# HorizonRobotics/HoloAgent

Measured on AMD Instinct MI355X. Metric: HMSG frames/sec (one scene per GPU: map A1-A2, fusion A3-A5, merge A6, pooling A7, floors A8, rooms by the device watershed N1, room clouds, room embeddings and View nodes A9, objects with the view <-> object test A10 and graph assembly A11, nothing handed in -- plus 1000 coarse-to-fine retrieval qu, higher is better.
Workload: dtype f64 geometry / f32 features

## Files before the change

### holoagent_amd/csrc/hmsg_merge.hip

```cpp
#include "hmsg_boundary.h"
#include "hmsg_cloudops.h"

#include <algorithm>
#include <cmath>
#include <numeric>
#include <chrono>
#include <unordered_map>
#include <condition_variable>
#include <deque>
#include <mutex>
#include <thread>

namespace {

struct Cloud {
    long long off = 0;
    int n = 0;
    double mn[3] = {0, 0, 0}, mx[3] = {0, 0, 0};
    bool fixed = false;
    bool fresh = true;
    bool raw = false;
    bool anchor = false;
    unsigned long long uid = 0;
    unsigned id = 0;
// ... 419 lines not shown
        if (lane == 0 && local) atomicAdd(&counts[npairs + lo], local);
    }
}

static const int CAT_CHUNK = 512;
__global__ void k_concat(const double* __restrict__ pool, const CatSeg* __restrict__ segs, int nsegs, double* __restrict__ dst,
                         const unsigned char* __restrict__ poolcore, unsigned char* __restrict__ dstcore, int chunk) {
    const CatSeg sg = segs[find_entry(segs, nsegs, blockIdx.x)];
    const long long p0 = (long long)(blockIdx.x - (unsigned)sg.blk0) * chunk, p1 = min((long long)sg.n, p0 + chunk);
    for (long long i = p0 * 3 + threadIdx.x; i < p1 * 3; i += blockDim.x) dst[sg.dst * 3 + i] = pool[sg.src * 3 + i];
    if (dstcore)
        for (long long i = p0 + threadIdx.x; i < p1; i += blockDim.x)
            dstcore[sg.dst + i] = sg.anchor ? poolcore[sg.src + i] : (unsigned char)0;
}

__host__ __device__ inline double box_iou(const double* amn, const double* amx, const double* bmn, const double* bmx) {
    if (amx[0] <= bmn[0] || bmx[0] <= amn[0] || amx[1] <= bmn[1] || bmx[1] <= amn[1] || amx[2] <= bmn[2] || bmx[2] <= amn[2])
        return 0.0;
    double ov = 1, va = 1, vb = 1;
    for (int k = 0; k < 3; ++k) {
        const double omin = amn[k] < bmn[k] ? bmn[k] : amn[k], omax = bmx[k] < amx[k] ? bmx[k] : amx[k];
        const double d = omax - omin;
        ov *= d < 0.0 ? 0.0 : d;
        va *= amx[k] - amn[k];
        vb *= bmx[k] - bmn[k];
    }
    return ov / (va + vb - ov);
}

static const int GP_TILE = 256;
struct GpTile {
    int row0, gend;
};
template <bool FILL>
__global__ void __launch_bounds__(GP_TILE) k_gp_pairs(const double* __restrict__ box, const GpTile* __restrict__ tiles, double iou_thresh, int n,
                                                      unsigned* __restrict__ cnt, const unsigned* __restrict__ start, int* __restrict__ out,
                                                      long long cap) {
    __shared__ double sb[GP_TILE * 6];
    const GpTile t = tiles[blockIdx.x];
    const int i = t.row0 + (int)threadIdx.x;
    const bool row = i < t.gend;
    double a[6] = {0, 0, 0, 0, 0, 0};
    if (row)
// ... 73 lines not shown
            h_out.ensure(2 + 2 * (size_t)cap_pairs);
        }
    }
    static bool fits(const int* group_off, int n_groups) {
        unsigned long long worst = 0;
        for (int g = 0; g < n_groups; ++g) {
            const unsigned long long m = (unsigned long long)(group_off[g + 1] - group_off[g]);
            worst += m * (m ? m - 1 : 0) / 2;
        }
        return worst < (1ull << 32);
    }
};

double bbox_iou(const Cloud& a, const Cloud& b) {
    return box_iou(a.mn, a.mx, b.mn, b.mx);
}

#define HMSG_BOX_MASK_BODY                                                                                          \
    for (int j = 0; j < n; ++j)                                                                                     \
        cm[j] = (unsigned char)!((q[1] <= lo0[j]) | (hi0[j] <= q[0]) | (q[3] <= lo1[j]) | (hi1[j] <= q[2]) |        \
                                 (q[5] <= lo2[j]) | (hi2[j] <= q[4]));
#if !defined(__HIP_DEVICE_COMPILE__) && defined(__x86_64__)
__attribute__((target("avx2"))) void box_mask_avx2(int n, const double* lo0, const double* hi0, const double* lo1,
                                                   const double* hi1, const double* lo2, const double* hi2, const double* q,
                                                   unsigned char* cm) {
    HMSG_BOX_MASK_BODY
}
#endif
void box_mask(int n, const double* lo0, const double* hi0, const double* lo1, const double* hi1, const double* lo2,
              const double* hi2, const double* q, unsigned char* cm) {
#if !defined(__HIP_DEVICE_COMPILE__) && defined(__x86_64__)
    static const bool have_avx2 = __builtin_cpu_supports("avx2");
    if (have_avx2) {
        box_mask_avx2(n, lo0, hi0, lo1, hi1, lo2, hi2, q, cm);
        return;
    }
#endif
    HMSG_BOX_MASK_BODY
}

struct IntSpan {
    const int* b;
    const int* e;
    size_t size() const { return (size_t)(e - b); }
    int operator[](size_t k) const { return b[k]; }
    const int* begin() const { return b; }
    const int* end() const { return e; }
};
struct CompList {
    std::vector<int> off, mem;
    size_t size() const { return off.empty() ? 0 : off.size() - 1; }
    IntSpan operator[](size_t c) const { return IntSpan{mem.data() + off[c], mem.data() + off[c + 1]}; }
};
// ... 304 lines not shown
        hipLaunchKernelGGL(k_ov_count, dim3(nblk), dim3(256), 0, s, (const double*)pool.p, (const OvGrid*)ds.p, (int)spec.size(),
                           d_cursor.p, ix_cells_used, OVI_CHUNK);
        HMSG_CHECK_LAUNCH();
        hmsg_scan_u32(d_cursor.p, ix_cells.p + ix_cells_used, (size_t)ncell_new, s, ops.scan_tmp, nullptr);
        hipLaunchKernelGGL(k_ov_fill, dim3(nblk), dim3(256), 0, s, (const double*)pool.p, (const OvGrid*)ds.p, (int)spec.size(),
                           (const unsigned*)ix_cells.p, d_cursor.p, ix_cells_used, ix_pts.p, OVI_CHUNK);
        HMSG_CHECK_LAUNCH();
    }

    void overlap_ratios(const std::vector<Cloud>& L, const std::vector<std::pair<int, int>>& pairs, std::vector<double>& ratio,
                        double decide_th, std::vector<unsigned char>* second_ran = nullptr) {
        ratio.assign(pairs.size(), 0.0);
        if (second_ran) second_ran->assign(pairs.size(), 0);
        if (pairs.empty()) return;
        const size_t P = pairs.size();
        std::vector<int> slot(L.size(), -1);
        std::vector<OvGrid> g;
        std::vector<OvTask> tasks(P * 2);
        unsigned nblk1 = 0, nblk2 = 0;
        for (size_t k = 0; k < P; ++k) {
            int a = pairs[k].first, b = pairs[k].second;
            for (int v : {a, b})
                if (slot[v] < 0) {
                    slot[v] = (int)g.size();
                    push_grids(L[v], g);
                }
            if (L[a].n > L[b].n) std::swap(a, b);
            tasks[k] = OvTask{slot[a], slot[b], 0, (int)nblk1};
            tasks[P + k] = OvTask{slot[b], slot[a], L[a].n, (int)nblk2};
            nblk1 += cdiv((size_t)L[a].n, OV_CHUNK);
            nblk2 += cdiv((size_t)L[b].n, OV_CHUNK);
        }
        for (size_t k = 0; k < P; ++k) tasks[P + k].blk0 += (int)nblk1;
// ... 5 lines not shown
        const size_t off_t = (g.size() * sizeof(OvGrid) + 15) & ~(size_t)15, off_c = off_t + tasks.size() * sizeof(OvTask),
                     off_b = off_c + tasks.size() * 4, pack = off_b + nblk_tab * 4;
        h_ovpack.ensure(pack);
        d_ovpack.ensure(pack);
        memcpy(h_ovpack.p, g.data(), g.size() * sizeof(OvGrid));
        memcpy(h_ovpack.p + off_t, tasks.data(), tasks.size() * sizeof(OvTask));
        memset(h_ovpack.p + off_c, 0, tasks.size() * 4);
        {
            int* bt = (int*)(h_ovpack.p + off_b);
            for (size_t k = 0; k < (plan ? P : 2 * P); ++k) {
                const size_t e = k + 1 < 2 * P ? (size_t)tasks[k + 1].blk0 : nblk;
                for (size_t b = (size_t)tasks[k].blk0; b < e; ++b) bt[b] = (int)k;
            }
        }
        upload_pinned(d_ovpack.p, h_ovpack.p, pack, s);
        const OvGrid* const dg = (const OvGrid*)d_ovpack.p;
        const OvTask* const dt = (const OvTask*)(d_ovpack.p + off_t);
        unsigned* const dc = (unsigned*)(d_ovpack.p + off_c);
        const int* const db = (const int*)(d_ovpack.p + off_b);
        const float r = (float)reach;
        const float r2 = (float)(radius * radius);
        const size_t prof_idx = ops.prof->ev.size();
        static const int ov_sorted_src = getenv("HMSG_OV_POOL_ORDER") == nullptr ? 1 : 0;
        unsigned long long* d_ovstat = nullptr;
        if (want_stats) {
            if (!ovstat.p) {
                ovstat.alloc(16);
                HIP_TRY(hipMemsetAsync(ovstat.p, 0, 128, s));
            }
            d_ovstat = ovstat.p;
// ... 73 lines not shown
                        gp_box[(size_t)i * 6 + a] = L[i].n ? L[i].mn[a] : 1e300;
                        gp_box[(size_t)i * 6 + 3 + a] = L[i].n ? L[i].mx[a] : -1e300;
                    }
                long long np = 0;
                const int* pr = gp.run(s, ops.scan_tmp, ops.prof, gp_box.data(), n, group_off->data(), G, iou_thresh, &np);
                for (long long k = 0; k < np; ++k) candidate(pr[2 * k], pr[2 * k + 1]);
            } else {
                for (int g = 0; g < G; ++g)
                    for (int i = (*group_off)[g]; i < (*group_off)[g + 1]; ++i)
                        for (int j = i + 1; j < (*group_off)[g + 1]; ++j) consider(i, j);
            }
        } else if (use_cache) {
            for (int i = 0; i < n; ++i)
                for (int j = i + 1; j < n; ++j) consider(i, j);
        } else {
            std::vector<double>* lo = fp_lo;
            std::vector<double>* hi = fp_hi;
            for (int a = 0; a < 3; ++a) {
                lo[a].resize((size_t)n);
                hi[a].resize((size_t)n);
            }
            fp_fr.resize((size_t)n);
            fp_cand.assign((size_t)n + 8, 0);
            std::vector<unsigned char>& fr = fp_fr;
            double u[6] = {1e300, -1e300, 1e300, -1e300, 1e300, -1e300};
            for (int j = 0; j < n; ++j) {
                fr[(size_t)j] = L[j].fresh ? 1 : 0;
                for (int a = 0; a < 3; ++a) {
                    lo[a][(size_t)j] = L[j].n ? L[j].mn[a] : 1e300;
                    hi[a][(size_t)j] = L[j].n ? L[j].mx[a] : -1e300;
                }
                if (fr[(size_t)j] && L[j].n)
                    for (int a = 0; a < 3; ++a) {
                        u[2 * a] = std::min(u[2 * a], L[j].mn[a]);
                        u[2 * a + 1] = std::max(u[2 * a + 1], L[j].mx[a]);
                    }
            }
            if (!(u[0] <= u[1])) return;
            box_mask(n, lo[0].data(), hi[0].data(), lo[1].data(), hi[1].data(), lo[2].data(), hi[2].data(), u, fp_cand.data());
            fp_sub.clear();
            for (int j = 0; j < n; ++j)
                if (fp_cand[(size_t)j]) fp_sub.push_back(j);
            const int m = (int)fp_sub.size();
            for (int a = 0; a < 3; ++a) {
                fp_slo[a].resize((size_t)m);
                fp_shi[a].resize((size_t)m);
                for (int q = 0; q < m; ++q) {
                    fp_slo[a][(size_t)q] = lo[a][(size_t)fp_sub[(size_t)q]];
                    fp_shi[a][(size_t)q] = hi[a][(size_t)fp_sub[(size_t)q]];
                }
            }
            fp_cand.assign((size_t)m + 8, 0);
            for (int i = 0; i < n; ++i) {
                if (!fr[(size_t)i] || L[i].n == 0) continue;
                unsigned char* cm = fp_cand.data();
                const double q[6] = {lo[0][(size_t)i], hi[0][(size_t)i], lo[1][(size_t)i], hi[1][(size_t)i], lo[2][(size_t)i], hi[2][(size_t)i]};
                box_mask(m, fp_slo[0].data(), fp_shi[0].data(), fp_slo[1].data(), fp_shi[1].data(), fp_slo[2].data(), fp_shi[2].data(), q, cm);
                for (int j0 = 0; j0 < m; j0 += 8) {
                    unsigned long long w;
                    std::memcpy(&w, cm + j0, 8);
                    if (!w) continue;
                    for (int jq = j0; jq < std::min(j0 + 8, m); ++jq) {
                        const int j = fp_sub[(size_t)jq];
                        if (!cm[jq] || j == i || (fr[(size_t)j] && j < i)) continue;
                        consider(std::min(i, j), std::max(i, j));
                    }
                }
            }
        }
    }
    GroupPairs gp;
    std::vector<double> gp_box;
    bool gp_wanted = getenv("HMSG_DEBUG_TREE_HOST_PAIRS") == nullptr;
    double gp_device_batches = 0, gp_host_batches = 0;
    std::vector<double> fp_lo[3], fp_hi[3], fp_slo[3], fp_shi[3];
    std::vector<unsigned char> fp_fr, fp_cand;
    std::vector<int> fp_sub;

    void make_components(const std::vector<Cloud>& L, const std::vector<std::pair<int, int>>& pairs, const std::vector<double>& ratio,
                         const std::vector<std::pair<int, int>>& known_pairs, const std::vector<double>& known, double th,
                         CompList& comps) {
        const int n = (int)L.size();
        std::vector<int> parent(n);
        std::iota(parent.begin(), parent.end(), 0);
        auto find = [&](int x) {
            while (parent[x] != x) x = parent[x] = parent[parent[x]];
            return x;
        };
        auto unite = [&](int a, int b) {
            a = find(a);
            b = find(b);
            if (a != b) parent[std::max(a, b)] = std::min(a, b);
        };
        for (size_t k = 0; k < pairs.size(); ++k) {
            if (use_cache) ratio_cache[L[pairs[k].first].uid * 0x100000000ull + L[pairs[k].second].uid] = ratio[k];
            if (ratio[k] > th) unite(pairs[k].first, pairs[k].second);
        }
        for (size_t k = 0; k < known_pairs.size(); ++k)
            if (known[k] > th) unite(known_pairs[k].first, known_pairs[k].second);
        {
            std::vector<int> comp_of(n, -1), cid(n);
            int nc = 0;
            for (int i = 0; i < n; ++i) {
                int r = find(i);
                if (comp_of[r] < 0) comp_of[r] = nc++;
                cid[i] = comp_of[r];
            }
            comps.off.assign((size_t)nc + 1, 0);
            for (int i = 0; i < n; ++i) ++comps.off[cid[i] + 1];
            for (int c = 0; c < nc; ++c) comps.off[c + 1] += comps.off[c];
            comps.mem.resize(n);
            std::vector<int> cur(comps.off.begin(), comps.off.end() - 1);
            for (int i = 0; i < n; ++i) comps.mem[cur[cid[i]]++] = i;
        }
    }

    std::vector<Cloud> merge_3d_masks(std::vector<Cloud> L, double th, const std::vector<int>* group_off = nullptr,
                                      std::vector<int>* out_group_off = nullptr) {
        const int n = (int)L.size();
        if (out_group_off) out_group_off->assign(group_off->size(), 0);
        if (n == 0) return L;
        auto tnow = [] { return std::chrono::steady_clock::now(); };
        auto t0 = tnow();
        auto lap = [&](int k) {
            auto t1 = tnow();
            tphase[k] += std::chrono::duration<double, std::milli>(t1 - t0).count();
            t0 = t1;
        };
        if (want_stats)
            for (auto& c : L) c.has_index_before = c.has_index;
        build_indices(L);
        lap(0);
        std::vector<std::pair<int, int>> pairs;
        std::vector<double> known;
        std::vector<std::pair<int, int>> known_pairs;
        find_pairs(L, pairs, known, known_pairs, group_off);
        std::vector<double> ratio;
        lap(1);
        std::vector<unsigned char> second_ran;
        overlap_ratios(L, pairs, ratio, use_cache ? -1.0 : th, want_stats ? &second_ran : nullptr);
        lap(2);
        if (want_stats) {
            st.steps += 1;
            st.clouds += n;
            for (int i = 0; i < n; ++i) {
                if (L[i].fresh && L[i].raw) st.fresh_raw += 1;
                if (L[i].fresh && !L[i].raw) st.fresh_g += 1;
                if (!L[i].has_index_before) st.idx_pts += L[i].n;
            }
            for (size_t k = 0; k < pairs.size(); ++k) {
                const Cloud &a = L[pairs[k].first], &b = L[pairs[k].second];
                const bool g = (a.fresh && !a.raw) || (b.fresh && !b.raw);
                const double n1 = std::min(a.n, b.n), n2 = second_ran[k] ? std::max(a.n, b.n) : 0;
                (g ? st.pairs_g : st.pairs_raw) += 1;
// ... 1 lines not shown
                (g ? st.scan2_g : st.scan2_raw) += n2;
            }
        }
        {
            static const char* const ovlog = getenv("HMSG_DEBUG_OVERLAP_LOG");
            if (ovlog && !pairs.empty()) {
                if (FILE* f = fopen(ovlog, "ab")) {
                    for (size_t k = 0; k < pairs.size(); ++k) {
                        const double rec[2] = {ratio[k], th};
                        fwrite(rec, 8, 2, f);
                    }
                    fclose(f);
                }
            }
        }
        CompList comps;
        make_components(L, pairs, ratio, known_pairs, known, th, comps);
        std::vector<int> seg_of_comp(comps.size(), -1);
        std::vector<SegDesc> segs;
        std::vector<int> seg_cap;
        long long region_total = 0;
        const bool inplace = use_anchor && inplace_wanted && CloudOps::regions_supported();
        std::vector<CatSeg> cat;
        long long cat_total = 0;
        unsigned cat_blocks = 0;
        for (size_t c = 0; c < comps.size(); ++c) {
            const auto& mem = comps[c];
            if (mem.size() == 1 && (L[mem[0]].fixed || L[mem[0]].n == 0)) continue;
            SegDesc sd;
            sd.pt_base = cat_total;
            sd.n = 0;
            bool any = false;
            int anchor_i = -1;
            if (use_anchor)
                for (int i : mem)
                    if (L[i].anchor && (anchor_i < 0 || L[i].n > L[anchor_i].n)) anchor_i = i;
            for (int i : mem) {
                if (L[i].n == 0) continue;
// ... 41 lines not shown
                        } else {
                            sd.out_mode = 1;
                            const long long cap = (long long)sd.n + std::max<long long>(sd.n / 2, 1 << 14);
                            sd.out_off = region_total;
                            region_total += cap;
                            HMSG_REQUIRE(cap <= 0x7fffffffll, HMSG_ERR_UNSUPPORTED, "merge fold: a merged cloud's pool region exceeds 2^31 points");
                            seg_cap.push_back((int)cap);
                        }
                    }
                }
            }
            if (seg_cap.size() <= segs.size()) seg_cap.push_back(0);
            seg_of_comp[c] = (int)segs.size();
            segs.push_back(sd);
        }
        std::vector<DbscanResult> res;
        long long dense_total = 0;
        for (auto& sd : segs) {
            if (sd.out_mode == 1) sd.out_off += pool_used;
            if (sd.out_mode == 0) dense_total += sd.n;
        }
        long long out_base = pool_used + region_total;
        if (!segs.empty() && cat_total > 0) {
            concat.ensure((size_t)cat_total * 3);
            concat_core.ensure((size_t)cat_total);
            grow(pool, (size_t)pool_used * 3, (size_t)(out_base + dense_total) * 3);
            grow(poolcore, (size_t)pool_used, (size_t)(out_base + dense_total));
            lap(3);
            DbGather ga;
            ga.pool = pool.p;
            ga.host_segs = cat.data();
            ga.nsegs = (int)cat.size();
            ga.poolcore = poolcore.p;
            ga.dstcore = use_anchor ? concat_core.p : nullptr;
            ga.pool_w = pool.p;
            ga.poolcore_w = poolcore.p;
            spec.clear();
            spec_of_seg.assign(segs.size(), -1);
            const bool speculate = spec_wanted && CloudOps::regions_supported();
            ops.dbscan_keep_largest(concat.p, segs, eps, minpts, pool.p + (size_t)out_base * 3, res,
                                    use_anchor ? (const unsigned char*)concat_core.p : nullptr, poolcore.p + out_base, &ga,
                                    speculate ? std::function<void(const unsigned*, int)>([&](const unsigned* d_res, int K) {
                                        speculate_indices(L, comps, seg_of_comp, segs, out_base, d_res, K);
                                    }) : std::function<void(const unsigned*, int)>());
            lap(4);
            if (want_stats) {
                for (size_t c = 0; c < comps.size(); ++c) {
                    if (seg_of_comp[c] < 0) continue;
                    const auto& mem = comps[c];
                    const DbscanResult& r = res[seg_of_comp[c]];
                    long long tot = 0, rest = 0;
                    bool rest_raw = true;
                    for (size_t q = 0; q < mem.size(); ++q) {
                        tot += L[mem[q]].n;
                        if (q) {
                            rest += L[mem[q]].n;
                            rest_raw = rest_raw && L[mem[q]].raw;
                        }
                    }
// ... 32 lines not shown
                    removed += segs[seg_of_comp[c]].n - r.n_out;
                    if (r.n_clusters > 1) {
                        ++multicl;
                        multicl_pts += r.n_out;
                        multicl_changed += r.changed;
                    }
                }
                fprintf(stderr, "[mstat] clouds %d pairs %zu segs %zu multi %d N %lld fixed_pts %lld anchor_pts %lld changed %d removed %lld multicl %d multicl_changed %d multicl_pts %lld\n",
                        n, pairs.size(), segs.size(), multi, cat_total, fixed_pts, big_fixed, nchanged, removed, multicl,
                        multicl_changed, multicl_pts);
            }
        } else {
            res.assign(segs.size(), DbscanResult{});
            spec.clear();
            spec_of_seg.assign(segs.size(), -1);
        }
        std::vector<int> spec_code(spec.size(), 0), spec_first(spec.size(), 0);
        std::vector<long long> spec_pt(spec.size(), 0);
        {
            long long pts = 0, cells_end = 0;
            for (size_t j = 0; j < spec.size(); ++j) {
                const DbscanResult& r = res[(size_t)spec[j].seg];
                int n_idx = 0;
                spec_code[j] = ov_spec_decide(spec[j], r.n_out, r.first_kept, &spec_first[j], &n_idx);
                spec_pt[j] = pts;
                pts += n_idx;
                if (n_idx > 0) {
                    cells_end = (spec[j].g.ix_cell - ix_cells_used) + spec[j].ncell;
                    spec_built += 1;
                    spec_built_pts += n_idx;
                    (spec_code[j] == 2 ? grid_delta : grid_full) += 1;
                    (spec_code[j] == 2 ? grid_delta_pts : grid_full_pts) += n_idx;
                } else {
                    spec_skipped += 1;
                }
            }
            for (size_t j = 0; j < spec.size(); ++j) spec_pt[j] = ix_pts_used;
            ix_cells_used += cells_end;
            ix_pts_used += pts;
        }
        std::vector<Cloud> out;
        out.reserve(comps.size());
        long long cursor = out_base;
        for (size_t c = 0; c < comps.size(); ++c) {
            const auto& mem = comps[c];
            int sg = seg_of_comp[c];
            if (sg < 0) {
                Cloud k = L[mem[0]];
                k.fresh = false;
                k.fixed = true;
                out.push_back(k);
                continue;
            }
            const DbscanResult& r = res[sg];
            if (mem.size() == 1 && !r.changed) {
                Cloud k = L[mem[0]];
                k.fresh = false;
                k.fixed = true;
                k.raw = false;
                k.off = cursor;
                k.cap = k.n;
                k.anchor = r.n_clusters == 1;
                out.push_back(k);
                cursor += r.n_out;
                continue;
            }
            Cloud k;
            const int mode = segs[sg].out_mode;
            k.off = mode ? segs[sg].out_off : cursor;
            k.cap = mode ? seg_cap[sg] : r.n_out;
            k.n = r.n_out;
            for (int a = 0; a < 3; ++a) {
                k.mn[a] = r.mn[a];
                k.mx[a] = r.mx[a];
            }
            k.fixed = !r.changed || r.n_clusters == 1 || (r.n_clusters > 1 && !r.contested);
            k.anchor = k.fixed && r.n_clusters >= 1 && (r.changed || r.n_clusters == 1);
            k.fresh = true;
// ... 25 lines not shown
                    k.gd2[0] = sp.g.gx, k.gd2[1] = sp.g.gy, k.gd2[2] = sp.g.gz;
                    for (int a = 0; a < 3; ++a) k.dmn[a] = (float)segs[sg].mn[a];
                }
                if (code == 3) {
                    k.nb = k.n;
                    k.ix_cell = sp.g.ix_cell;
                    k.ix_pt = spec_pt[(size_t)sj];
                    k.gd[0] = sp.g.gx, k.gd[1] = sp.g.gy, k.gd[2] = sp.g.gz;
                    for (int a = 0; a < 3; ++a) k.bmn[a] = (float)segs[sg].mn[a];
                }
                k.has_index = code != 0;
            } else if (inherit_grids && r.first_kept >= 0 && f >= 0 && r.first_kept == L[f].n && L[f].has_index && L[f].nb > 0) {
                take_base();
                k.has_index = k.nb == k.n;
            }
            out.push_back(k);
            if (!mode) cursor += r.n_out;
        }
        pool_used = cursor;
        if (out_group_off) {
            const int G = (int)group_off->size() - 1;
            size_t c = 0;
            for (int g = 0; g < G; ++g) {
                (*out_group_off)[(size_t)g] = (int)c;
                while (c < comps.size() && comps[c][0] < (*group_off)[(size_t)g + 1]) ++c;
            }
            (*out_group_off)[(size_t)G] = (int)c;
        }
        lap(5);
        return out;
    }
};

}
// ... 183 lines not shown
    fprintf(stderr, "[hmsg fold] steps %.0f  components: anchor %.0f  plain %.0f  batch %.0f   active points %.0f  relocated %.0f   ids %u\n",
            m.fstat[0], m.fstat[1], m.fstat[2], m.fstat[3], m.fstat[4], m.fstat[5], m.next_id);
    unsigned cnt[FC_N];
    HIP_TRY(hipMemcpy(cnt, m.ix_counters.p, sizeof(cnt), hipMemcpyDeviceToHost));
    fprintf(stderr, "[hmsg fold] index: %u of %u bricks, %u of %u records, hash %u slots\n", cnt[FC_BRICKS], m.ix.brick_cap, cnt[FC_RECS],
            m.ix.rec_cap, m.ix.hmask + 1);
    fprintf(stderr, "[hmsg fold] point pool: %lld points in use (%.2f GB), %lld in the frame masks\n", m.pool_used, m.pool_used * 25e-9, (long long)h->masks3d.total);
    fprintf(stderr, "[hmsg fold] walks: count %u  touch %u  link %u  label %u   touched anchor points %u\n", cnt[FC_STAT], cnt[FC_STAT + 1],
            cnt[FC_STAT + 2], cnt[FC_STAT + 3], cnt[FC_STAT + 4]);
    fprintf(stderr, "[hmsg fold] link walks: anchor comps own %u promoted %u raw %u | plain comps own %u promoted %u raw %u\n", cnt[FC_DBG], cnt[FC_DBG + 1],
            cnt[FC_DBG + 2], cnt[FC_DBG + 4], cnt[FC_DBG + 5], cnt[FC_DBG + 6]);
}

static void merge_report(Folder& m) {
    if (getenv("HMSG_DEBUG_TIMING"))
        fprintf(stderr, "[hmsg merge] index %.1f  pairs(host) %.1f  overlap %.1f  components+concat %.1f  dbscan %.1f  bookkeeping %.1f ms\n",
                m.tphase[0], m.tphase[1], m.tphase[2], m.tphase[3], m.tphase[4], m.tphase[5]);
    if (m.want_stats) {
        const auto& t = m.st;
        const double S = std::max(1.0, t.steps);
        fprintf(stderr, "[mstat] steps %.0f  per step: clouds %.1f  fresh raw %.1f  fresh G %.1f  indexed pts %.0f\n", t.steps, t.clouds / S,
                t.fresh_raw / S, t.fresh_g / S, t.idx_pts / S);
        fprintf(stderr, "[mstat] pairs/step raw %.1f (scan1 %.0f scan2 %.0f pts)   G-fresh %.1f (scan1 %.0f scan2 %.0f pts)\n", t.pairs_raw / S,
                t.scan1_raw / S, t.scan2_raw / S, t.pairs_g / S, t.scan1_g / S, t.scan2_g / S);
        if (m.ovstat.p) {
            unsigned long long hs[16];
            (void)hipMemcpy(hs, m.ovstat.p, 128, hipMemcpyDeviceToHost);
            fprintf(stderr, "[mstat] overlap probes with > 32 candidates: %.1f per step, %.0f candidates per step; longest candidate list of a probe %llu\n",
                    hs[8] / S, hs[9] / S, hs[7]);
            fprintf(stderr, "[mstat] overlap probes/step %.0f: outside the box %.0f  hit own cell %.0f  hit neighbour %.0f  miss %.0f | candidates/step own %.0f  neighbour %.0f\n",
                    hs[0] / S, hs[1] / S, hs[2] / S, hs[3] / S, hs[4] / S, hs[5] / S, hs[6] / S);
        }
// ... 32 lines not shown
    bool incremental = false, never = false;
    int f_switch = -1;
    double batch_mean = 0.0, switch_points = 1500000.0;

    void init(hmsg_ctx* hh, hipStream_t stream, Prof* prof) {
        h = hh;
        merger_init(m, h);
        m.s = stream;
        m.ops.s = stream;
        m.ops.prof = prof;
        if (const char* e = getenv("HMSG_DEBUG_GC_POINTS")) m.gc_pool_points = (size_t)atoll(e);
        never = getenv("HMSG_FOLD_LEGACY") != nullptr;
        switch_points = getenv("HMSG_FOLD_INCREMENTAL") ? 0.0 : 1500000.0;
        if (const char* e = getenv("HMSG_FOLD_SWITCH")) switch_points = atof(e);
        if (const char* e = getenv("HMSG_FOLD_BIG_ACTIVE")) m.big_active = atoll(e);
    }
    void ingest(const double* src, long long npts, const long long* off, const std::vector<int>& nm, long long reserve) {
        if (m.pool.n == 0) {
            m.pool.alloc((size_t)std::max<long long>(npts * reserve, 1 << 16) * 3);
            m.poolcore.alloc((size_t)std::max<long long>(npts * reserve, 1 << 16));
        } else {
            m.grow(m.pool, (size_t)m.pool_used * 3, (size_t)(m.pool_used + npts) * 3);
            m.grow(m.poolcore, (size_t)m.pool_used, (size_t)(m.pool_used + npts));
        }
        const long long base = m.pool_used;
        if (npts) HIP_TRY(hipMemcpyAsync(m.pool.p + (size_t)base * 3, src, (size_t)npts * 24, hipMemcpyDeviceToDevice, m.s));
        m.pool_used += npts;
        size_t nmask = 0;
        for (int v : nm) nmask += (size_t)v;
        std::vector<SegDesc> msegs(nmask);
// ... 38 lines not shown
            batch_mean += (last_batch - batch_mean) / 64.0;
            if (input_complete && (switch_points <= 0.0 || batch_mean > switch_points) && fold_begin(m, h, G, frames, f)) {
                incremental = true;
                f_switch = (int)f;
            }
        }
        if (incremental) {
            G.insert(G.end(), frames[f].begin(), frames[f].end());
            std::vector<Cloud>().swap(frames[f]);
            G = m.fold_step(std::move(G), c.init_overlap_thresh);
            return;
        }
        if (m.needs_collect()) {
            m.collect(G, frames, f);
            prebuilt_upto = f;
        }
        if (f >= prebuilt_upto) {
            const size_t b = std::min(frames.size(), f + Merger::PREBUILD_WINDOW);
            m.prebuild(frames, f, b);
            prebuilt_upto = b;
        }
        G.insert(G.end(), frames[f].begin(), frames[f].end());
        std::vector<Cloud>().swap(frames[f]);
        G = m.merge_3d_masks(std::move(G), c.init_overlap_thresh);
    }
    void finish() {
        const hmsg_config& c = h->cfg;
        std::vector<Cloud> result = incremental ? m.fold_step(std::move(G), c.init_overlap_thresh) : m.merge_3d_masks(std::move(G), c.init_overlap_thresh);
        if (getenv("HMSG_DEBUG_TIMING") && incremental) {
            fprintf(stderr, "[hmsg merge] incremental fold from frame %d of %zu\n", f_switch, frames.size());
            fold_report(m, h);
        }
        store_instances(m, h, result, c.min_instance_points);
        merge_report(m);
    }
};

struct FoldPipe {
// ... 567 lines not shown
```

Measured before the change: 2667.

## Plan next frame's merge pairs ahead while the device DBSCAN runs

Moves the box table and candidate pair enumeration into a persistent FoldPlan. After each merge step the table is updated in place, and pairs involving the next frame's masks are enumerated inside the DBSCAN callback so the host work overlaps device execution. At the next step only pairs involving the changed components are computed late and merged into the precomputed list. It also reuses workspace vectors across steps instead of reallocating them. The added complexity risks pair ordering and correctness subtleties, and ahead plans must be dropped when a collect happens.

After: 2714 (median of 6 runs). +1.8%, better.

```diff
diff --git a/holoagent_amd/csrc/hmsg_fold_host.h b/holoagent_amd/csrc/hmsg_fold_host.h
--- /dev/null
+++ b/holoagent_amd/csrc/hmsg_fold_host.h
@@ -0,0 +1,268 @@
+#pragma once
+
+#include <algorithm>
+#include <cstring>
+#include <utility>
+#include <vector>
+
+#if defined(__HIPCC__)
+#define HMSG_FOLD_HD __host__ __device__
+#else
+#define HMSG_FOLD_HD
+#endif
+
+HMSG_FOLD_HD inline double box_iou(const double* amn, const double* amx, const double* bmn, const double* bmx) {
+    if (amx[0] <= bmn[0] || bmx[0] <= amn[0] || amx[1] <= bmn[1] || bmx[1] <= amn[1] || amx[2] <= bmn[2] || bmx[2] <= amn[2])
+        return 0.0;
+    double ov = 1, va = 1, vb = 1;
+    for (int k = 0; k < 3; ++k) {
+        const double omin = amn[k] < bmn[k] ? bmn[k] : amn[k], omax = bmx[k] < amx[k] ? bmx[k] : amx[k];
+        const double d = omax - omin;
+        ov *= d < 0.0 ? 0.0 : d;
+        va *= amx[k] - amn[k];
+        vb *= bmx[k] - bmn[k];
+    }
+    return ov / (va + vb - ov);
+}
+
+#define HMSG_BOX_MASK_BODY                                                                                          \
+    for (int j = 0; j < n; ++j)                                                                                     \
+        cm[j] = (unsigned char)!((q[1] <= lo0[j]) | (hi0[j] <= q[0]) | (q[3] <= lo1[j]) | (hi1[j] <= q[2]) |        \
+                                 (q[5] <= lo2[j]) | (hi2[j] <= q[4]));
+#if !defined(__HIP_DEVICE_COMPILE__) && defined(__x86_64__)
+__attribute__((target("avx2"))) inline void box_mask_avx2(int n, const double* lo0, const double* hi0, const double* lo1,
+                                                          const double* hi1, const double* lo2, const double* hi2, const double* q,
+                                                          unsigned char* cm) {
+    HMSG_BOX_MASK_BODY
+}
+#endif
+inline void box_mask(int n, const double* lo0, const double* hi0, const double* lo1, const double* hi1, const double* lo2,
+                     const double* hi2, const double* q, unsigned char* cm) {
+#if !defined(__HIP_DEVICE_COMPILE__) && defined(__x86_64__)
+    static const bool have_avx2 = __builtin_cpu_supports("avx2");
+    if (have_avx2) {
+        box_mask_avx2(n, lo0, hi0, lo1, hi1, lo2, hi2, q, cm);
+        return;
+    }
+#endif
+    HMSG_BOX_MASK_BODY
+}
+
+typedef std::vector<std::pair<int, int>> FoldPairList;
+
+struct FoldBoxTable {
+    std::vector<double> lo[3], hi[3];
+    std::vector<unsigned char> fresh;
+    std::vector<int> np;
+    int n = 0;
+    void resize(int m) {
+        for (int a = 0; a < 3; ++a) {
+            lo[a].resize((size_t)m);
+            hi[a].resize((size_t)m);
+        }
+        fresh.resize((size_t)m);
+        np.resize((size_t)m);
+        n = m;
+    }
+    void set(int i, const double* mn, const double* mx, int points, bool fr) {
+        for (int a = 0; a < 3; ++a) {
+            lo[a][(size_t)i] = points ? mn[a] : 1e300;
+            hi[a][(size_t)i] = points ? mx[a] : -1e300;
+        }
+        np[(size_t)i] = points;
+        fresh[(size_t)i] = fr ? 1 : 0;
+    }
+    void move(int dst, int src) {
+        for (int a = 0; a < 3; ++a) {
+            lo[a][(size_t)dst] = lo[a][(size_t)src];
+            hi[a][(size_t)dst] = hi[a][(size_t)src];
+        }
+        np[(size_t)dst] = np[(size_t)src];
+        fresh[(size_t)dst] = fresh[(size_t)src];
+    }
+    bool same(int i, const FoldBoxTable& o, int j) const {
+        for (int a = 0; a < 3; ++a)
+            if (lo[a][(size_t)i] != o.lo[a][(size_t)j] || hi[a][(size_t)i] != o.hi[a][(size_t)j]) return false;
+        return np[(size_t)i] == o.np[(size_t)j] && fresh[(size_t)i] == o.fresh[(size_t)j];
+    }
+    double iou(int i, int j) const {
+        const double amn[3] = {lo[0][(size_t)i], lo[1][(size_t)i], lo[2][(size_t)i]}, amx[3] = {hi[0][(size_t)i], hi[1][(size_t)i], hi[2][(size_t)i]};
+        const double bmn[3] = {lo[0][(size_t)j], lo[1][(size_t)j], lo[2][(size_t)j]}, bmx[3] = {hi[0][(size_t)j], hi[1][(size_t)j], hi[2][(size_t)j]};
+        return box_iou(amn, amx, bmn, bmx);
+    }
+};
+
+struct FoldPairScratch {
+    std::vector<double> slo[3], shi[3];
+    std::vector<unsigned char> cand;
+    std::vector<int> sub, from;
+};
+
+inline void fold_pairs_from(const FoldBoxTable& t, const int* from, int nfrom, double iou_thresh, FoldPairScratch& s, FoldPairList& pairs,
+                            std::vector<int>* from_off = nullptr) {
+    const int n = t.n;
+    if (from_off) from_off->assign((size_t)nfrom + 1, (int)pairs.size());
+    if (nfrom == 0) return;
+    double u[6] = {1e300, -1e300, 1e300, -1e300, 1e300, -1e300};
+    for (int k = 0; k < nfrom; ++k)
+        for (int a = 0; a < 3; ++a) {
+            u[2 * a] = std::min(u[2 * a], t.lo[a][(size_t)from[k]]);
+            u[2 * a + 1] = std::max(u[2 * a + 1], t.hi[a][(size_t)from[k]]);
+        }
+    s.cand.assign((size_t)n + 8, 0);
+    box_mask(n, t.lo[0].data(), t.hi[0].data(), t.lo[1].data(), t.hi[1].data(), t.lo[2].data(), t.hi[2].data(), u, s.cand.data());
+    s.sub.clear();
+    for (int j = 0; j < n; ++j)
+        if (s.cand[(size_t)j]) s.sub.push_back(j);
+    const int m = (int)s.sub.size();
+    for (int a = 0; a < 3; ++a) {
+        s.slo[a].resize((size_t)m);
+        s.shi[a].resize((size_t)m);
+        for (int q = 0; q < m; ++q) {
+            s.slo[a][(size_t)q] = t.lo[a][(size_t)s.sub[(size_t)q]];
+            s.shi[a][(size_t)q] = t.hi[a][(size_t)s.sub[(size_t)q]];
+        }
+    }
+    s.cand.assign((size_t)m + 8, 0);
+    for (int k = 0; k < nfrom; ++k) {
+        const int i = from[k];
+        if (from_off) (*from_off)[(size_t)k] = (int)pairs.size();
+        unsigned char* cm = s.cand.data();
+        const double q[6] = {t.lo[0][(size_t)i], t.hi[0][(size_t)i], t.lo[1][(size_t)i], t.hi[1][(size_t)i], t.lo[2][(size_t)i], t.hi[2][(size_t)i]};
+        box_mask(m, s.slo[0].data(), s.shi[0].data(), s.slo[1].data(), s.shi[1].data(), s.slo[2].data(), s.shi[2].data(), q, cm);
+        for (int j0 = 0; j0 < m; j0 += 8) {
+            unsigned long long w;
+            std::memcpy(&w, cm + j0, 8);
+            if (!w) continue;
+            for (int jq = j0; jq < std::min(j0 + 8, m); ++jq) {
+                const int j = s.sub[(size_t)jq];
+                if (!cm[jq] || j == i || (t.fresh[(size_t)j] && j < i)) continue;
+                if (t.np[(size_t)i] == 0 || t.np[(size_t)j] == 0) continue;
+                if (!(t.iou(i, j) > iou_thresh)) continue;
+                pairs.emplace_back(std::min(i, j), std::max(i, j));
+            }
+        }
+    }
+    if (from_off) (*from_off)[(size_t)nfrom] = (int)pairs.size();
+}
+
+inline void fold_pairs_reference(const FoldBoxTable& t, double iou_thresh, FoldPairScratch& s, FoldPairList& pairs) {
+    s.from.clear();
+    for (int i = 0; i < t.n; ++i)
+        if (t.fresh[(size_t)i] && t.np[(size_t)i]) s.from.push_back(i);
+    fold_pairs_from(t, s.from.data(), (int)s.from.size(), iou_thresh, s, pairs);
+}
+
+template <class List>
+inline void fold_fill_boxes(const List& L, int first, FoldBoxTable& t) {
+    t.resize((int)L.size());
+    for (int j = first; j < (int)L.size(); ++j) t.set(j, L[(size_t)j].mn, L[(size_t)j].mx, L[(size_t)j].n, L[(size_t)j].fresh);
+}
+
+template <class List>
+inline void fold_keep_untouched(List& L, size_t c, size_t src) {
+    if (src != c) L[c] = L[src];
+    L[c].fresh = false;
+    L[c].fixed = true;
+}
+
+struct FoldPlan {
+    FoldBoxTable tab;
+    bool synced = false;
+    bool ahead = false;
+    int n_out = 0;
+    std::vector<int> pending;
+    int n_resolved = 0;
+    FoldPairList apairs;
+    std::vector<int> aoff;
+    FoldPairScratch scratch;
+    std::vector<int> unchanged;
+    double n_ahead_steps = 0, n_late_only_steps = 0;
+
+    void reset() {
+        synced = ahead = false;
+        tab.n = 0;
+        n_out = 0;
+        pending.clear();
+        n_resolved = 0;
+    }
+    void drop_ahead() {
+        if (!ahead) return;
+        ahead = false;
+        tab.resize(n_out);
+    }
+    void advance(const int* comp_off, const int* comp_mem, int nc, const int* seg_of_comp) {
+        pending.clear();
+        n_resolved = 0;
+        static const double z[3] = {0, 0, 0};
+        for (int c = 0; c < nc; ++c) {
+            if (seg_of_comp[c] < 0) {
+                const int src = comp_mem[comp_off[c]];
+                if (src != c) tab.move(c, src);
+                tab.fresh[(size_t)c] = 0;
+            } else {
+                tab.set(c, z, z, 0, false);
+                pending.push_back(c);
+            }
+        }
+        tab.resize(nc);
+        n_out = nc;
+        synced = true;
+        ahead = false;
+    }
+    void append(const double* mn, const double* mx, int points) {
+        tab.resize(tab.n + 1);
+        tab.set(tab.n - 1, mn, mx, points, true);
+    }
+    void plan_ahead(double iou_thresh) {
+        scratch.from.clear();
+        for (int i = n_out; i < tab.n; ++i) scratch.from.push_back(i);
+        apairs.clear();
+        fold_pairs_from(tab, scratch.from.data(), (int)scratch.from.size(), iou_thresh, scratch, apairs, &aoff);
+        ahead = true;
+    }
+    void resolve(int c, const double* mn, const double* mx, int points, bool fr) {
+        tab.set(c, mn, mx, points, fr);
+        ++n_resolved;
+    }
+    bool resolved() const { return n_resolved == (int)pending.size(); }
+    template <class List>
+    void step_pairs(const List& L, double iou_thresh, FoldPairList& pairs) {
+        const int n = (int)L.size();
+        if (synced && ahead && tab.n == n && resolved()) {
+            pairs_late(iou_thresh, pairs);
+            n_ahead_steps += 1;
+            return;
+        }
+        const bool keep = synced && !ahead && resolved() && tab.n <= n;
+        fold_fill_boxes(L, keep ? tab.n : 0, tab);
+        fold_pairs_reference(tab, iou_thresh, scratch, pairs);
+        n_late_only_steps += 1;
+    }
+    void pairs_late(double iou_thresh, FoldPairList& pairs) {
+        scratch.from.clear();
+        unchanged.clear();
+        for (int c : pending) {
+            if (tab.np[(size_t)c] == 0) continue;
+            (tab.fresh[(size_t)c] ? scratch.from : unchanged).push_back(c);
+        }
+        fold_pairs_from(tab, scratch.from.data(), (int)scratch.from.size(), iou_thresh, scratch, pairs);
+        const int nm = tab.n - n_out;
+        if (unchanged.empty()) {
+            pairs.insert(pairs.end(), apairs.begin(), apairs.end());
+            return;
+        }
+        for (int k = 0; k < nm; ++k) {
+            const int i = n_out + k;
+            size_t pa = (size_t)aoff[(size_t)k];
+            const size_t pe = (size_t)aoff[(size_t)k + 1];
+            if (tab.np[(size_t)i])
+                for (int u : unchanged) {
+                    if (!(tab.iou(i, u) > iou_thresh)) continue;
+                    while (pa < pe && apairs[pa].second == i && apairs[pa].first < u) pairs.push_back(apairs[pa++]);
+                    pairs.emplace_back(u, i);
+                }
+            pairs.insert(pairs.end(), apairs.begin() + (long)pa, apairs.begin() + (long)pe);
+        }
+    }
+};
diff --git a/holoagent_amd/csrc/hmsg_merge.hip b/holoagent_amd/csrc/hmsg_merge.hip
--- a/holoagent_amd/csrc/hmsg_merge.hip
+++ b/holoagent_amd/csrc/hmsg_merge.hip
@@ -1,5 +1,6 @@
 #include "hmsg_boundary.h"
 #include "hmsg_cloudops.h"
+#include "hmsg_fold_host.h"
 
 #include <algorithm>
 #include <cmath>
@@ -457,19 +458,6 @@
             dstcore[sg.dst + i] = sg.anchor ? poolcore[sg.src + i] : (unsigned char)0;
 }
 
-__host__ __device__ inline double box_iou(const double* amn, const double* amx, const double* bmn, const double* bmx) {
-    if (amx[0] <= bmn[0] || bmx[0] <= amn[0] || amx[1] <= bmn[1] || bmx[1] <= amn[1] || amx[2] <= bmn[2] || bmx[2] <= amn[2])
-        return 0.0;
-    double ov = 1, va = 1, vb = 1;
-    for (int k = 0; k < 3; ++k) {
-        const double omin = amn[k] < bmn[k] ? bmn[k] : amn[k], omax = bmx[k] < amx[k] ? bmx[k] : amx[k];
-        const double d = omax - omin;
-        ov *= d < 0.0 ? 0.0 : d;
-        va *= amx[k] - amn[k];
-        vb *= bmx[k] - bmn[k];
-    }
-    return ov / (va + vb - ov);
-}
 
 static const int GP_TILE = 256;
 struct GpTile {
@@ -573,29 +561,6 @@
 
 double bbox_iou(const Cloud& a, const Cloud& b) {
     return box_iou(a.mn, a.mx, b.mn, b.mx);
-}
-
-#define HMSG_BOX_MASK_BODY                                                                                          \
-    for (int j = 0; j < n; ++j)                                                                                     \
-        cm[j] = (unsigned char)!((q[1] <= lo0[j]) | (hi0[j] <= q[0]) | (q[3] <= lo1[j]) | (hi1[j] <= q[2]) |        \
-                                 (q[5] <= lo2[j]) | (hi2[j] <= q[4]));
-#if !defined(__HIP_DEVICE_COMPILE__) && defined(__x86_64__)
-__attribute__((target("avx2"))) void box_mask_avx2(int n, const double* lo0, const double* hi0, const double* lo1,
-                                                   const double* hi1, const double* lo2, const double* hi2, const double* q,
-                                                   unsigned char* cm) {
-    HMSG_BOX_MASK_BODY
-}
-#endif
-void box_mask(int n, const double* lo0, const double* hi0, const double* lo1, const double* hi1, const double* lo2,
-              const double* hi2, const double* q, unsigned char* cm) {
-#if !defined(__HIP_DEVICE_COMPILE__) && defined(__x86_64__)
-    static const bool have_avx2 = __builtin_cpu_supports("avx2");
-    if (have_avx2) {
-        box_mask_avx2(n, lo0, hi0, lo1, hi1, lo2, hi2, q, cm);
-        return;
-    }
-#endif
-    HMSG_BOX_MASK_BODY
 }
 
 struct IntSpan {
@@ -930,9 +895,13 @@
         if (second_ran) second_ran->assign(pairs.size(), 0);
         if (pairs.empty()) return;
         const size_t P = pairs.size();
-        std::vector<int> slot(L.size(), -1);
-        std::vector<OvGrid> g;
-        std::vector<OvTask> tasks(P * 2);
+        const auto pack_t0 = std::chrono::steady_clock::now();
+        std::vector<int>& slot = ws_slot;
+        std::vector<OvGrid>& g = ws_grids;
+        std::vector<OvTask>& tasks = ws_tasks;
+        slot.assign(L.size(), -1);
+        g.clear();
+        tasks.resize(P * 2);
         unsigned nblk1 = 0, nblk2 = 0;
         for (size_t k = 0; k < P; ++k) {
             int a = pairs[k].first, b = pairs[k].second;
@@ -968,6 +937,7 @@
             }
         }
         upload_pinned(d_ovpack.p, h_ovpack.p, pack, s);
+        t_ovpack += std::chrono::duration<double, std::milli>(std::chrono::steady_clock::now() - pack_t0).count();
         const OvGrid* const dg = (const OvGrid*)d_ovpack.p;
         const OvTask* const dt = (const OvTask*)(d_ovpack.p + off_t);
         unsigned* const dc = (unsigned*)(d_ovpack.p + off_c);
@@ -1071,74 +1041,56 @@
             for (int i = 0; i < n; ++i)
                 for (int j = i + 1; j < n; ++j) consider(i, j);
         } else {
-            std::vector<double>* lo = fp_lo;
-            std::vector<double>* hi = fp_hi;
-            for (int a = 0; a < 3; ++a) {
-                lo[a].resize((size_t)n);
-                hi[a].resize((size_t)n);
-            }
-            fp_fr.resize((size_t)n);
-            fp_cand.assign((size_t)n + 8, 0);
-            std::vector<unsigned char>& fr = fp_fr;
-            double u[6] = {1e300, -1e300, 1e300, -1e300, 1e300, -1e300};
-            for (int j = 0; j < n; ++j) {
-                fr[(size_t)j] = L[j].fresh ? 1 : 0;
-                for (int a = 0; a < 3; ++a) {
-                    lo[a][(size_t)j] = L[j].n ? L[j].mn[a] : 1e300;
-                    hi[a][(size_t)j] = L[j].n ? L[j].mx[a] : -1e300;
-                }
-                if (fr[(size_t)j] && L[j].n)
-                    for (int a = 0; a < 3; ++a) {
-                        u[2 * a] = std::min(u[2 * a], L[j].mn[a]);
-                        u[2 * a + 1] = std::max(u[2 * a + 1], L[j].mx[a]);
-                    }
-            }
-            if (!(u[0] <= u[1])) return;
-            box_mask(n, lo[0].data(), hi[0].data(), lo[1].data(), hi[1].data(), lo[2].data(), hi[2].data(), u, fp_cand.data());
-            fp_sub.clear();
-            for (int j = 0; j < n; ++j)
-                if (fp_cand[(size_t)j]) fp_sub.push_back(j);
-            const int m = (int)fp_sub.size();
-            for (int a = 0; a < 3; ++a) {
-                fp_slo[a].resize((size_t)m);
-                fp_shi[a].resize((size_t)m);
-                for (int q = 0; q < m; ++q) {
-                    fp_slo[a][(size_t)q] = lo[a][(size_t)fp_sub[(size_t)q]];
-                    fp_shi[a][(size_t)q] = hi[a][(size_t)fp_sub[(size_t)q]];
-                }
-            }
-            fp_cand.assign((size_t)m + 8, 0);
-            for (int i = 0; i < n; ++i) {
-                if (!fr[(size_t)i] || L[i].n == 0) continue;
-                unsigned char* cm = fp_cand.data();
-                const double q[6] = {lo[0][(size_t)i], hi[0][(size_t)i], lo[1][(size_t)i], hi[1][(size_t)i], lo[2][(size_t)i], hi[2][(size_t)i]};
-                box_mask(m, fp_slo[0].data(), fp_shi[0].data(), fp_slo[1].data(), fp_shi[1].data(), fp_slo[2].data(), fp_shi[2].data(), q, cm);
-                for (int j0 = 0; j0 < m; j0 += 8) {
-                    unsigned long long w;
-                    std::memcpy(&w, cm + j0, 8);
-                    if (!w) continue;
-                    for (int jq = j0; jq < std::min(j0 + 8, m); ++jq) {
-                        const int j = fp_sub[(size_t)jq];
-                        if (!cm[jq] || j == i || (fr[(size_t)j] && j < i)) continue;
-                        consider(std::min(i, j), std::max(i, j));
-                    }
-                }
-            }
+            fold_fill_boxes(L, 0, fp_tab);
+            fold_pairs_reference(fp_tab, iou_thresh, fp_scratch, pairs);
         }
     }
     GroupPairs gp;
     std::vector<double> gp_box;
     bool gp_wanted = getenv("HMSG_DEBUG_TREE_HOST_PAIRS") == nullptr;
     double gp_device_batches = 0, gp_host_batches = 0;
-    std::vector<double> fp_lo[3], fp_hi[3], fp_slo[3], fp_shi[3];
-    std::vector<unsigned char> fp_fr, fp_cand;
-    std::vector<int> fp_sub;
+    FoldBoxTable fp_tab;
+    FoldPairScratch fp_scratch;
+    std::vector<std::pair<int, int>> ws_pairs, ws_known_pairs;
+    std::vector<double> ws_known, ws_ratio;
+    std::vector<unsigned char> ws_second_ran;
+    CompList ws_comps;
+    std::vector<int> ws_seg_of_comp, ws_seg_cap, ws_spec_code, ws_spec_first, ws_parent, ws_comp_of, ws_cid, ws_cur;
+    std::vector<long long> ws_spec_pt;
+    std::vector<int> ws_slot;
+    std::vector<OvGrid> ws_grids;
+    std::vector<OvTask> ws_tasks;
+    std::vector<SegDesc> ws_segs;
+    std::vector<CatSeg> ws_cat;
+    std::vector<DbscanResult> ws_res;
+    FoldPlan plan;
+    bool plan_wanted = false;
+    bool plan_enabled = !(getenv("HMSG_FOLD_HOST_AHEAD") && atoi(getenv("HMSG_FOLD_HOST_AHEAD")) == 0);
+    bool plan_check = getenv("HMSG_DEBUG_FOLD_PAIRS_CHECK") != nullptr && atoi(getenv("HMSG_DEBUG_FOLD_PAIRS_CHECK")) != 0;
+    const std::vector<Cloud>* next_masks = nullptr;
+    double t_ovpack = 0;
+    double t_ahead_hidden = 0;
+    FoldPairList chk_pairs;
+    void planned_pairs(const std::vector<Cloud>& L, FoldPairList& pairs) {
+        const int n = (int)L.size();
+        plan.step_pairs(L, iou_thresh, pairs);
+        if (plan_check) {
+            fold_fill_boxes(L, 0, fp_tab);
+            chk_pairs.clear();
+            fold_pairs_reference(fp_tab, iou_thresh, fp_scratch, chk_pairs);
+            bool same = plan.tab.n == n;
+            for (int i = 0; same && i < n; ++i) same = plan.tab.same(i, fp_tab, i);
+            HMSG_REQUIRE(same, HMSG_ERR_INVALID, "merge fold: the kept box table differs from the cloud list");
+            HMSG_REQUIRE(pairs == chk_pairs, HMSG_ERR_INVALID, "merge fold: the planned pair list differs from the reference enumerator's");
+        }
+    }
 
     void make_components(const std::vector<Cloud>& L, const std::vector<std::pair<int, int>>& pairs, const std::vector<double>& ratio,
                          const std::vector<std::pair<int, int>>& known_pairs, const std::vector<double>& known, double th,
                          CompList& comps) {
         const int n = (int)L.size();
-        std::vector<int> parent(n);
+        std::vector<int>& parent = ws_parent;
+        parent.resize((size_t)n);
         std::iota(parent.begin(), parent.end(), 0);
         auto find = [&](int x) {
             while (parent[x] != x) x = parent[x] = parent[parent[x]];
@@ -1156,7 +1108,9 @@
         for (size_t k = 0; k < known_pairs.size(); ++k)
             if (known[k] > th) unite(known_pairs[k].first, known_pairs[k].second);
         {
-            std::vector<int> comp_of(n, -1), cid(n);
+            std::vector<int>&comp_of = ws_comp_of, &cid = ws_cid, &cur = ws_cur;
+            comp_of.assign((size_t)n, -1);
+            cid.resize((size_t)n);
             int nc = 0;
             for (int i = 0; i < n; ++i) {
                 int r = find(i);
@@ -1167,7 +1121,7 @@
             for (int i = 0; i < n; ++i) ++comps.off[cid[i] + 1];
             for (int c = 0; c < nc; ++c) comps.off[c + 1] += comps.off[c];
             comps.mem.resize(n);
-            std::vector<int> cur(comps.off.begin(), comps.off.end() - 1);
+            cur.assign(comps.off.begin(), comps.off.end() - 1);
             for (int i = 0; i < n; ++i) comps.mem[cur[cid[i]]++] = i;
         }
     }
@@ -1186,15 +1140,22 @@
         };
         if (want_stats)
             for (auto& c : L) c.has_index_before = c.has_index;
+        const bool planned = plan_wanted && plan_enabled && !use_cache && !group_off;
+        const std::vector<Cloud>* const masks_ahead = planned ? next_masks : nullptr;
+        next_masks = nullptr;
         build_indices(L);
         lap(0);
-        std::vector<std::pair<int, int>> pairs;
-        std::vector<double> known;
-        std::vector<std::pair<int, int>> known_pairs;
-        find_pairs(L, pairs, known, known_pairs, group_off);
-        std::vector<double> ratio;
+        std::vector<std::pair<int, int>>& pairs = ws_pairs;
+        std::vector<double>& known = ws_known;
+        std::vector<std::pair<int, int>>& known_pairs = ws_known_pairs;
+        pairs.clear();
+        known.clear();
+        known_pairs.clear();
+        if (planned) planned_pairs(L, pairs);
+        else find_pairs(L, pairs, known, known_pairs, group_off);
+        std::vector<double>& ratio = ws_ratio;
         lap(1);
-        std::vector<unsigned char> second_ran;
+        std::vector<unsigned char>& second_ran = ws_second_ran;
         overlap_ratios(L, pairs, ratio, use_cache ? -1.0 : th, want_stats ? &second_ran : nullptr);
         lap(2);
         if (want_stats) {
@@ -1226,14 +1187,18 @@
                 }
             }
         }
-        CompList comps;
+        CompList& comps = ws_comps;
         make_components(L, pairs, ratio, known_pairs, known, th, comps);
-        std::vector<int> seg_of_comp(comps.size(), -1);
-        std::vector<SegDesc> segs;
-        std::vector<int> seg_cap;
+        std::vector<int>& seg_of_comp = ws_seg_of_comp;
+        seg_of_comp.assign(comps.size(), -1);
+        std::vector<SegDesc>& segs = ws_segs;
+        std::vector<int>& seg_cap = ws_seg_cap;
+        segs.clear();
+        seg_cap.clear();
         long long region_total = 0;
         const bool inplace = use_anchor && inplace_wanted && CloudOps::regions_supported();
-        std::vector<CatSeg> cat;
+        std::vector<CatSeg>& cat = ws_cat;
+        cat.clear();
         long long cat_total = 0;
         unsigned cat_blocks = 0;
         for (size_t c = 0; c < comps.size(); ++c) {
@@ -1305,7 +1270,25 @@
             seg_of_comp[c] = (int)segs.size();
             segs.push_back(sd);
         }
-        std::vector<DbscanResult> res;
+        std::vector<DbscanResult>& res = ws_res;
+        bool advanced = false;
+        auto advance_plan = [&](bool hidden) {
+            if (!planned || advanced) return;
+            advanced = true;
+            const auto a0 = tnow();
+            plan.advance(comps.off.data(), comps.mem.data(), (int)comps.size(), seg_of_comp.data());
+            if (masks_ahead) {
+                for (const Cloud& c : *masks_ahead) plan.append(c.mn, c.mx, c.n);
+                plan.plan_ahead(iou_thresh);
+            }
+            const auto a1 = tnow();
+            if (hidden) {
+                t_ahead_hidden += std::chrono::duration<double, std::milli>(a1 - a0).count();
+            } else {
+                tphase[1] += std::chrono::duration<double, std::milli>(a1 - a0).count();
+                t0 += a1 - a0;
+            }
+        };
         long long dense_total = 0;
         for (auto& sd : segs) {
             if (sd.out_mode == 1) sd.out_off += pool_used;
@@ -1331,9 +1314,11 @@
             const bool speculate = spec_wanted && CloudOps::regions_supported();
             ops.dbscan_keep_largest(concat.p, segs, eps, minpts, pool.p + (size_t)out_base * 3, res,
                                     use_anchor ? (const unsigned char*)concat_core.p : nullptr, poolcore.p + out_base, &ga,
-                                    speculate ? std::function<void(const unsigned*, int)>([&](const unsigned* d_res, int K) {
-                                        speculate_indices(L, comps, seg_of_comp, segs, out_base, d_res, K);
+                                    (speculate || planned) ? std::function<void(const unsigned*, int)>([&](const unsigned* d_res, int K) {
+                                        if (speculate) speculate_indices(L, comps, seg_of_comp, segs, out_base, d_res, K);
+                                        advance_plan(true);
                                     }) : std::function<void(const unsigned*, int)>());
+            advance_plan(false);
             lap(4);
             if (want_stats) {
                 for (size_t c = 0; c < comps.size(); ++c) {
@@ -1396,9 +1381,13 @@
             res.assign(segs.size(), DbscanResult{});
             spec.clear();
             spec_of_seg.assign(segs.size(), -1);
-        }
-        std::vector<int> spec_code(spec.size(), 0), spec_first(spec.size(), 0);
-        std::vector<long long> spec_pt(spec.size(), 0);
+            advance_plan(false);
+        }
+        std::vector<int>&spec_code = ws_spec_code, &spec_first = ws_spec_first;
+        std::vector<long long>& spec_pt = ws_spec_pt;
+        spec_code.assign(spec.size(), 0);
+        spec_first.assign(spec.size(), 0);
+        spec_pt.assign(spec.size(), 0);
         {
             long long pts = 0, cells_end = 0;
             for (size_t j = 0; j < spec.size(); ++j) {
@@ -1422,11 +1411,23 @@
             ix_pts_used += pts;
         }
         std::vector<Cloud> out;
-        out.reserve(comps.size());
+        if (!planned) out.reserve(comps.size());
+        auto put = [&](size_t c, const Cloud& k) {
+            if (planned) {
+                L[c] = k;
+                plan.resolve((int)c, k.mn, k.mx, k.n, k.fresh);
+            } else {
+                out.push_back(k);
+            }
+        };
         long long cursor = out_base;
         for (size_t c = 0; c < comps.size(); ++c) {
             const auto& mem = comps[c];
             int sg = seg_of_comp[c];
+            if (sg < 0 && planned) {
+                fold_keep_untouched(L, c, (size_t)mem[0]);
+                continue;
+            }
             if (sg < 0) {
                 Cloud k = L[mem[0]];
                 k.fresh = false;
@@ -1443,7 +1444,7 @@
                 k.off = cursor;
                 k.cap = k.n;
                 k.anchor = r.n_clusters == 1;
-                out.push_back(k);
+                put(c, k);
                 cursor += r.n_out;
                 continue;
             }
@@ -1499,10 +1500,16 @@
                 take_base();
                 k.has_index = k.nb == k.n;
             }
-            out.push_back(k);
+            put(c, k);
             if (!mode) cursor += r.n_out;
         }
         pool_used = cursor;
+        if (planned) {
+            HMSG_REQUIRE(plan.resolved(), HMSG_ERR_INVALID, "merge fold: an output of the step was not entered into the box table");
+            L.resize(comps.size());
+            lap(5);
+            return L;
+        }
         if (out_group_off) {
             const int G = (int)group_off->size() - 1;
             size_t c = 0;
@@ -1716,8 +1723,11 @@
 
 static void merge_report(Folder& m) {
     if (getenv("HMSG_DEBUG_TIMING"))
-        fprintf(stderr, "[hmsg merge] index %.1f  pairs(host) %.1f  overlap %.1f  components+concat %.1f  dbscan %.1f  bookkeeping %.1f ms\n",
-                m.tphase[0], m.tphase[1], m.tphase[2], m.tphase[3], m.tphase[4], m.tphase[5]);
+        fprintf(stderr, "[hmsg merge] index %.1f  pairs(host) late (on the chain) %.1f  ahead (hidden) %.1f  overlap %.1f (pack fill %.1f)  components+concat %.1f  dbscan %.1f  bookkeeping %.1f ms\n",
+                m.tphase[0], m.tphase[1], m.t_ahead_hidden, m.tphase[2], m.t_ovpack, m.tphase[3], m.tphase[4], m.tphase[5]);
+    if (getenv("HMSG_DEBUG_TIMING") && m.plan_wanted)
+        fprintf(stderr, "[hmsg merge] pair lists: %.0f steps merged from an ahead and a late part, %.0f enumerated whole after the results\n",
+                m.plan.n_ahead_steps, m.plan.n_late_only_steps);
     if (m.want_stats) {
         const auto& t = m.st;
         const double S = std::max(1.0, t.steps);
@@ -1780,6 +1790,7 @@
         switch_points = getenv("HMSG_FOLD_INCREMENTAL") ? 0.0 : 1500000.0;
         if (const char* e = getenv("HMSG_FOLD_SWITCH")) switch_points = atof(e);
         if (const char* e = getenv("HMSG_FOLD_BIG_ACTIVE")) m.big_active = atoll(e);
+        m.plan_wanted = true;
     }
     void ingest(const double* src, long long npts, const long long* off, const std::vector<int>& nm, long long reserve) {
         if (m.pool.n == 0) {
@@ -1848,6 +1859,7 @@
         if (m.needs_collect()) {
             m.collect(G, frames, f);
             prebuilt_upto = f;
+            m.plan.drop_ahead();
         }
         if (f >= prebuilt_upto) {
             const size_t b = std::min(frames.size(), f + Merger::PREBUILD_WINDOW);
@@ -1856,6 +1868,7 @@
         }
         G.insert(G.end(), frames[f].begin(), frames[f].end());
         std::vector<Cloud>().swap(frames[f]);
+        m.next_masks = f + 1 < frames.size() ? &frames[f + 1] : nullptr;
         G = m.merge_3d_masks(std::move(G), c.init_overlap_thresh);
     }
     void finish() {
```
